# kylegrover/raymarch-algo-compare

Measured on AMD Instinct MI355X. Metric: Mrays/sec (mean iters/ray alongside), 1920x1080 Mandelbulb/Standard, higher is better.
Workload: dtype f64

## Files before the change

raymarch_algo_compare_amd/csrc/rm_kernels.h:

```cpp
#pragma once

#define RM_TABLES_IN_LDS 1

#include <hip/hip_runtime.h>
#include <stdint.h>
#include <type_traits>

#include "rm_camera.h"
#include "rm_capture.h"
#include "rm_scenes.h"
#include "rm_shape.h"
#include "rm_strategies.h"

namespace rm {

constexpr int kHistBins = 544;
constexpr int kStatsHead = 24;
constexpr int kStatsWords = kStatsHead + kHistBins;
constexpr int kQueues = 2;
constexpr int kStatsParts = 64;
constexpr int kStatsBlocks = 1 + kStatsParts;

struct FrameParams {
    CameraParams cam;
// ... 615 lines not shown
            continue;
        }

        bool park = false;
        bool consume = active;
        if constexpr (INTERLEAVE) consume = active && ready;
        if (!INTERLEAVE || __any(consume)) {
            if (consume) {
                double d;
                if constexpr (INTERLEAVE) d = Scene::value(ev);
                else d = Scene::sdf(origin + dir * s.te);
                ++nev;
            if (s.step(d, cfg)) {
                    active = false;
                    const int it = s.res.iters, h = s.res.hit;
                    a.depth[my_gi] = h ? (float)s.res.t : 0.0f;
                    a.iters[my_gi] = it;
                    a.hit[my_gi] = (uint8_t)h;
                    if (raw_out) store_raw(a, my_gi, s.res, nev);
                    acc.evals += (unsigned)nev;
                    acc.add(it, h);
                    atomicAdd(&s_hist[min(it, a.hist_bins - 1)], 1u);
                    if (a.tile_cost) {
                        const uint32_t frame = my_gi / frame_elems;
                        const uint32_t pix = my_gi - frame * frame_elems;
                        const uint32_t y = pix / (uint32_t)a.width, x = pix - y * (uint32_t)a.width;
                        atomicMax(&a.tile_cost[frame * (uint32_t)a.tiles_per_frame + (y / 4u) * (uint32_t)a.tiles_x + (x >> 6)], it);
                    }
                } else if (a.suspend_after > 0 && s.i >= a.suspend_after) {
                    park = true;
                } else if constexpr (INTERLEAVE) {
                    ready = Scene::begin(ev, origin + dir * s.te);
                }
            }
            if (a.suspend_after > 0 && __any(park)) {
                const bool parked = push_suspended(a, a.suspend_queue, park, my_gi, s, nev);
                if (parked) {
                    active = false;
                } else if (park) {
                    if constexpr (INTERLEAVE) ready = Scene::begin(ev, origin + dir * s.te);
                }
            }
        }
        if constexpr (INTERLEAVE) {
            if (active && !ready) ready = Scene::trip(ev);
        }
    }

    unsigned long long* const part = stats_part(a.stats);
    acc.flush(part);
    __syncthreads();
    for (int b = threadIdx.x; b < kHistBins; b += blockDim.x) {
        const unsigned int c = s_hist[b];
        if (c) atomicAdd(&part[kStatsHead + b], (unsigned long long)c);
    }
}


template <class Scene>
__global__ __launch_bounds__(256) void sdf_eval_kernel(const double* __restrict__ xyz, size_t n, double* __restrict__ out, const void* scene_data)
{
    rm_load_scene_data<Scene>(scene_data);
    rm_load_tables<Scene>();
    size_t i = (size_t)blockIdx.x * blockDim.x + threadIdx.x;
    if (i < n) out[i] = Scene::sdf(v3(xyz[3 * i], xyz[3 * i + 1], xyz[3 * i + 2]));
}

template <class Scene, class Strat>
__global__ __launch_bounds__(64) void march_rays_kernel(MarchCfg cfg, const double* __restrict__ origins, const double* __restrict__ dirs,
                                  size_t n, uint8_t* hit, double* t, int32_t* iters, double* final_sdf, const void* scene_data)
{
    rm_load_scene_data<Scene>(scene_data);
    rm_load_tables<Scene>();
    size_t i = (size_t)blockIdx.x * blockDim.x + threadIdx.x;
    if (i >= n) return;
    vec3 o = v3(origins[3 * i], origins[3 * i + 1], origins[3 * i + 2]);
    vec3 d = normalized(v3(dirs[3 * i], dirs[3 * i + 1], dirs[3 * i + 2]));
    Result r = march_one<Scene, Strat>(o, d, cfg);
    hit[i] = (uint8_t)r.hit; t[i] = r.t; iters[i] = r.iters; final_sdf[i] = r.final_sdf;
}

constexpr int kTeam = 3;

struct TeamXch {
    double v[2][2 * kTeam][64];
};

template <class Scene, class PartT>
__device__ __forceinline__ bool team_trip(typename Scene::Eval& ev, bool go, PartT part, int lane, TeamXch& x, int& turn)
{
    double o0 = 0.0, o1 = 0.0;
    if constexpr (std::is_same<PartT, int>::value) {
        if (go) Scene::trip_part(ev, part, o0, o1);
    } else {
        if (go) Scene::template trip_part<PartT::value>(ev, o0, o1);
    }
    double (*buf)[64] = x.v[turn & 1];
    ++turn;
    buf[2 * (int)part][lane] = o0;
    buf[2 * (int)part + 1][lane] = o1;
    __syncthreads();
    bool done = true;
    if (go) done = Scene::trip_join(ev, buf[0][lane], buf[1][lane], buf[2][lane], buf[3][lane], buf[4][lane], buf[5][lane]);
    return done;
}

template <class Scene, class = void>
struct ScenePartLoops : std::false_type {};
template <class Scene>
struct ScenePartLoops<Scene, decltype((void)Scene::kPartLoops)> : std::integral_constant<bool, Scene::kPartLoops> {};

template <int P, class Trip>
__device__ __forceinline__ void team_trips_part(bool& ready, const Trip& trip)
{
    while (__any(!ready)) {
        const bool fin = trip(std::integral_constant<int, P>(), !ready);
        if (!ready) ready = fin;
    }
}
template <class Scene, class Trip>
__device__ __forceinline__ void team_trips(int part, bool& ready, const Trip& trip)
{
    if constexpr (ScenePartLoops<Scene>::value) {
        part = __builtin_amdgcn_readfirstlane(part);
        if (part == 0) team_trips_part<0>(ready, trip);
        else if (part == 1) team_trips_part<1>(ready, trip);
        else team_trips_part<2>(ready, trip);
    } else {
        while (__any(!ready)) {
            const bool fin = trip(part, !ready);
            if (!ready) ready = fin;
        }
    }
}

template <class Scene, class Strat>
__global__ __launch_bounds__(64 * kTeam) void march_rays_team_kernel(MarchCfg cfg, const double* __restrict__ origins,
                                                                     const double* __restrict__ dirs, size_t n, uint8_t* hit,
                                                                     double* t, int32_t* iters, double* final_sdf,
                                                                     unsigned long long* busy)
{
    __shared__ TeamXch xch;
    const unsigned int nteams = (unsigned int)((n + 63) / 64);
    if (blockIdx.x >= nteams) {
        if (busy) keep_busy_until(busy, (unsigned long long)nteams, 256);
        return;
    }
    rm_load_tables<Scene>();
    const int lane = lane_id();
    const int part = (int)(threadIdx.x >> 6);
    const size_t i = (size_t)blockIdx.x * 64 + (size_t)lane;
    const bool have = i < n;
    vec3 o = v3(0.0, 0.0, 0.0), d = v3(0.0, 0.0, 1.0);
    if (have) {
        o = v3(origins[3 * i], origins[3 * i + 1], origins[3 * i + 2]);
        d = normalized(v3(dirs[3 * i], dirs[3 * i + 1], dirs[3 * i + 2]));
    }
    Strat s;
    bool done = true;
    if (have) done = s.start(cfg);
    typename Scene::Eval ev;
    int turn = 0;
    while (__any(!done)) {
        bool ready = true;
        if (!done) ready = Scene::begin(ev, o + d * s.te);
        team_trips<Scene>(part, ready, [&](auto P, bool go) { return team_trip<Scene>(ev, go, P, lane, xch, turn); });
        if (!done) done = s.step(Scene::value(ev), cfg);
    }
    if (have && part == 0) {
        hit[i] = (uint8_t)s.res.hit; t[i] = s.res.t; iters[i] = s.res.iters; final_sdf[i] = s.res.final_sdf;
    }
    if (busy && threadIdx.x == 0) __hip_atomic_fetch_add(busy, 1ull, __ATOMIC_RELAXED, __HIP_MEMORY_SCOPE_AGENT);
}

template <class Scene, class Strat, bool BATCH>
__global__ __launch_bounds__(64 * kTeam) void resume_team_kernel(const KernelArgs a, const int level)
{
    using Entry = QEntry<Strat>;
    __shared__ TeamXch xch;
    __shared__ unsigned int s_hist[kHistBins];
    __shared__ unsigned int s_base;
    const int lane = lane_id();
    const int part = (int)(threadIdx.x >> 6);
    for (int b = threadIdx.x; b < kHistBins; b += blockDim.x) s_hist[b] = 0u;
    rm_load_tables<Scene>();
    __syncthreads();

    const unsigned long long pushed = a.stats[6 + level];
    const unsigned int count = (unsigned int)min(pushed, (unsigned long long)a.queue_cap);
    const Entry* const queue = (const Entry*)a.queue[level];
    const uint32_t frame_elems = (uint32_t)a.rows * (uint32_t)a.width;
    if (a.keep_busy > 0 && (int)blockIdx.x >= a.team_wgs) {
        const unsigned long long t0 = __builtin_amdgcn_s_memrealtime();
        while (__hip_atomic_load(&a.stats[8 + level], __ATOMIC_RELAXED, __HIP_MEMORY_SCOPE_AGENT) < (unsigned long long)count &&
               __builtin_amdgcn_s_memrealtime() - t0 < 3000000ull)
            __builtin_amdgcn_s_sleep(127);
        keep_busy_until(&a.stats[12 + level], (unsigned long long)a.team_wgs, a.keep_busy);
        return;
    }

    WaveAcc acc;
    bool more = count > 0;
    bool active = false;
    uint32_t my_gi = 0;
    int nev = 0;
    vec3 origin = v3(0.0, 0.0, 0.0), dir = v3(0.0, 0.0, 0.0);
    MarchCfg lane_cfg = a.single.cfg;
    int raw_out = a.raw_outputs;
    pin_lane(raw_out);
    if constexpr (!BATCH) pin_cfg(lane_cfg);
    const MarchCfg& cfg = lane_cfg;
    Strat s;
    typename Scene::Eval ev;
    int turn = 0;

    for (;;) {
        const unsigned long long idle = __ballot(!active);
        const int nidle = __popcll(idle);
        if (more && (nidle >= a.refill_min || nidle == 64)) {
            if (part == 0 && lane == 0) s_base = (unsigned int)atomicAdd(&a.stats[8 + level], (unsigned long long)nidle);
            __syncthreads();
            const unsigned int base = (unsigned int)__builtin_amdgcn_readfirstlane((int)s_base);
            __syncthreads();
            if (base >= count) {
                more = false;
            } else if (!active) {
                const unsigned int idx = base + (unsigned int)rank_in_mask(idle);
                if (idx < count) {
                    const Entry e = queue[idx];
                    my_gi = e.gi;
                    s = e.s;
                    nev = (int)e.nev;
                    const uint32_t frame = my_gi / frame_elems;
                    const uint32_t pix = my_gi - frame * frame_elems;
                    const int y = (int)(pix / (uint32_t)a.width);
                    const int x = (int)(pix - (uint32_t)y * (uint32_t)a.width);
                    const int gy = band_row(a, y);
                    if constexpr (BATCH) {
                        const FrameParams& fp = a.frames[frame];
                        camera_ray(fp.cam, a.width, a.height, x, gy, origin, dir);
                        lane_cfg = fp.cfg;
                        lane_cfg.full = a.full;
                    } else {
                        camera_ray(a.single.cam, a.width, a.height, x, gy, origin, dir);
                    }
                    active = true;
                }
            }
        }
        if (!__any(active)) {
            if (!more) break;
            continue;
        }

        bool ready = true;
        if (active) ready = Scene::begin(ev, origin + dir * s.te);
        team_trips<Scene>(part, ready, [&](auto P, bool go) { return team_trip<Scene>(ev, go, P, lane, xch, turn); });
        bool park = false;
        if (active) {
            ++nev;
            if (!s.step(Scene::value(ev), cfg)) {
                park = a.suspend_after > 0 && s.i >= a.suspend_after;
            } else {
            active = false;
            if (part == 0) {
                const int it = s.res.iters, h = s.res.hit;
                a.depth[my_gi] = h ? (float)s.res.t : 0.0f;
                a.iters[my_gi] = it;
                a.hit[my_gi] = (uint8_t)h;
                if (raw_out) store_raw(a, my_gi, s.res, nev);
                acc.evals += (unsigned)nev;
                acc.add(it, h);
                atomicAdd(&s_hist[min(it, a.hist_bins - 1)], 1u);
                if (a.tile_cost) {
                    const uint32_t frame = my_gi / frame_elems;
                    const uint32_t pix = my_gi - frame * frame_elems;
                    const uint32_t y = pix / (uint32_t)a.width, x = pix - y * (uint32_t)a.width;
                    atomicMax(&a.tile_cost[frame * (uint32_t)a.tiles_per_frame + (y / 4u) * (uint32_t)a.tiles_x + (x >> 6)], it);
                }
            }
            }
        }
        if (a.suspend_after > 0 && __any(park)) {
            const unsigned long long m = __ballot(park);
            if (part == 0 && lane == 0) {
                const unsigned long long b64 = atomicAdd(&a.stats[6 + a.suspend_queue], (unsigned long long)__popcll(m));
                s_base = b64 > 0xffffff00ull ? 0xffffff00u : (unsigned int)b64;
            }
            __syncthreads();
            const unsigned int base = (unsigned int)__builtin_amdgcn_readfirstlane((int)s_base);
            __syncthreads();
            const unsigned long long idx = (unsigned long long)base + (unsigned long long)rank_in_mask(m);
            if (park && idx < (unsigned long long)a.queue_cap) {
                if (part == 0) {
                    Entry* e = (Entry*)a.queue[a.suspend_queue] + idx;
                    e->gi = my_gi;
                    e->nev = (uint32_t)nev;
                    e->s = s;
                }
                active = false;
            }
        }
    }

    unsigned long long* const spart = stats_part(a.stats);
    if (part == 0) acc.flush(spart);
    __syncthreads();
    for (int b = threadIdx.x; b < kHistBins; b += blockDim.x) {
        const unsigned int c = s_hist[b];
        if (c) atomicAdd(&spart[kStatsHead + b], (unsigned long long)c);
    }
    if (a.keep_busy > 0 && threadIdx.x == 0) __hip_atomic_fetch_add(&a.stats[12 + level], 1ull, __ATOMIC_RELAXED, __HIP_MEMORY_SCOPE_AGENT);
}

struct CaptureArgs {
    CameraParams cam;
    const CameraParams* cams;
    int32_t width, height, row0, rows;
    int32_t max_iterations;
    double max_distance;
    const uint8_t* hit;
    const double* t;
    const float* depth_in;
    const int32_t* iters;
    const double* final_sdf;
    const int32_t* evals;
    float* geom;
    float* normal;
    float* depth;
    float* color;
    float* evals_f;
    const void* scene_data;
};

template <class Scene> struct CaptureTables {};
template <class Scene> struct SceneTables<CaptureTables<Scene>> { static constexpr unsigned value = SceneTables<Scene>::value | TB_POW; };

template <class Scene>
__global__ __launch_bounds__(256) void capture_kernel(CaptureArgs a)
{
    rm_load_scene_data<Scene>(a.scene_data);
    rm_load_tables<CaptureTables<Scene>>();
    const size_t n = (size_t)a.rows * (size_t)a.width;
    const size_t i = (size_t)blockIdx.x * blockDim.x + threadIdx.x;
// ... 38 lines not shown
```

raymarch_algo_compare_amd/csrc/rm_pipeline.h:

```cpp
#pragma once

#include "rm_kernels.h"

namespace rm {

constexpr int kCtlStride = 16;
constexpr int kCTile = 0;
constexpr int kCReserved = 1;
constexpr int kCTaken = 3;
constexpr int kCFreshDone = 5;
constexpr int kCProdExited = 6;
constexpr int kCLeft = 7;
constexpr int kCLateStarted = 8;
constexpr int kCTeamDone = 9;
constexpr int kCtlWords = 10 * kCtlStride;
__device__ __forceinline__ unsigned long long* ctl(const KernelArgs& a, int k) { return a.ctl + k * kCtlStride; }
constexpr int kWMarkStart = 13;
constexpr int kWMarkFresh = 14;
constexpr int kWMarkProd = 15;
constexpr int kWMarkTiles = 17;
constexpr int kWMarkPush = 18;
constexpr int kWMarkPop = 19;
constexpr int kWLongPushMax = 20;
constexpr int kWLongTeamMax = 21;
// ... 55 lines not shown
            }
        }
    }
    __builtin_amdgcn_fence(__ATOMIC_ACQUIRE, "agent");
    return ok;
}

template <class Strat>
__device__ __forceinline__ bool q_push(const KernelArgs& a, int q, bool want, uint32_t gi, const Strat& s, int nev)
{
    const unsigned long long m = __ballot(want);
    if (m == 0) return false;
    unsigned long long base = 0;
    if (lane_id() == 0)
        base = __hip_atomic_fetch_add(ctl(a, kCReserved + q), (unsigned long long)__popcll(m), __ATOMIC_RELAXED,
                                      __HIP_MEMORY_SCOPE_AGENT);
    base = ((unsigned long long)(unsigned)__builtin_amdgcn_readfirstlane((int)(base >> 32)) << 32) |
           (unsigned)__builtin_amdgcn_readfirstlane((int)base);
    const unsigned long long idx = base + (unsigned long long)rank_in_mask(m);
    const bool ok = want && idx < (unsigned long long)a.queue_cap;
    static_assert(sizeof(QEntry<Strat>) % 8 == 0 && alignof(QEntry<Strat>) == 8, "entries are copied as 8-byte words");
    constexpr int NW = (int)(sizeof(QEntry<Strat>) / 8);
    constexpr int NP = (NW + 1) / 2;
    unsigned long long* const dst = (unsigned long long*)((QEntry<Strat>*)a.queue[q] + (ok ? idx : 0ull));
    unsigned long long w[NW];
    {
        QEntry<Strat> e;
        e.gi = gi;
        e.nev = (uint32_t)nev;
        e.ready = 0u;
        e.pad = a.marks ? (uint32_t)(realtime() - ~ld_relaxed(&a.stats[kWMarkStart])) : 0u;
        e.s = s;
        __builtin_memcpy(w, &e, sizeof e);
    }
    const int lane = lane_id();
    for (unsigned long long mm = __ballot(ok); mm != 0; mm &= mm - 1) {
        const int src = (int)__builtin_ctzll(mm);
        const unsigned int ilo = (unsigned int)__builtin_amdgcn_readlane((int)(unsigned int)idx, src);
        const unsigned int ihi = (unsigned int)__builtin_amdgcn_readlane((int)(unsigned int)(idx >> 32), src);
        unsigned int p0 = 0, p1 = 0, p2 = 0, p3 = 0;
#pragma unroll
        for (int p = 0; p < NP; ++p) {
            const unsigned int a0 = (unsigned int)__builtin_amdgcn_readlane((int)(unsigned int)w[2 * p], src);
            const unsigned int a1 = (unsigned int)__builtin_amdgcn_readlane((int)(unsigned int)(w[2 * p] >> 32), src);
            unsigned int a2 = 0, a3 = 0;
            if (2 * p + 1 < NW) {
                a2 = (unsigned int)__builtin_amdgcn_readlane((int)(unsigned int)w[2 * p + 1], src);
                a3 = (unsigned int)__builtin_amdgcn_readlane((int)(unsigned int)(w[2 * p + 1] >> 32), src);
            }
            if (lane == p) { p0 = a0; p1 = a1; p2 = a2; p3 = a3; }
        }
        char* const d = (char*)((QEntry<Strat>*)a.queue[q] + (((unsigned long long)ihi << 32) | ilo)) + 16 * lane;
        static_assert(std::is_base_of<StratBase, Strat>::value && __builtin_offsetof(StratBase, res) == 32 && sizeof(Result) == 24 &&
                      sizeof(QEntry<StratBase>) - sizeof(StratBase) == 16, "entry pieces 3 and 4 hold the result record");
        const bool dead = !a.full && (lane == 3 || (NW == 9 && lane == 4));
        if (lane < NP && !dead) {
            if ((NW & 1) && lane == NP - 1) {
                __hip_atomic_store((unsigned long long*)d, ((unsigned long long)p1 << 32) | p0, __ATOMIC_RELAXED, __HIP_MEMORY_SCOPE_AGENT);
            } else {
                typedef unsigned int u32x4 __attribute__((ext_vector_type(4)));
                const u32x4 v = { p0, p1, p2, p3 };
                asm volatile("global_store_dwordx4 %0, %1, off sc1" ::"v"(d), "v"(v) : "memory");
            }
        }
    }
    asm volatile("s_waitcnt vmcnt(0)" ::: "memory");
    if (ok) __hip_atomic_store((uint32_t*)(dst + 1), a.generation, __ATOMIC_RELAXED, __HIP_MEMORY_SCOPE_AGENT);
    if (a.marks && q == 1 && lane_id() == 0) atomicMax(&a.stats[kWMarkPush], realtime());
    return ok;
}


template <int TILE_PIX>
struct PipeProducerLds {
    float depth[kPipeWaves][kSlots][TILE_PIX];
    uint32_t ih[kPipeWaves][kSlots][TILE_PIX];
};
struct PipeTeamLds {
    TeamXch xch;
    unsigned int hist[kHistBins];
    unsigned int base, count, queue, done;
    unsigned int ok_lo, ok_hi;
};

__device__ __forceinline__ void store_direct(const KernelArgs& a, uint32_t gi, const Result& r, int nev, WaveAcc& acc,
                                             unsigned int* s_hist)
{
    const int it = r.iters, h = r.hit;
    a.depth[gi] = h ? (float)r.t : 0.0f;
    a.iters[gi] = it;
    a.hit[gi] = (uint8_t)h;
    if (a.raw_outputs) store_raw(a, gi, r, nev);
    acc.evals += (unsigned)nev;
    acc.add(it, h);
    atomicAdd(&s_hist[min(it, a.hist_bins - 1)], 1u);
    if (a.tile_cost) {
        const uint32_t frame_elems = (uint32_t)a.rows * (uint32_t)a.width;
        const uint32_t frame = gi / frame_elems;
        const uint32_t pix = gi - frame * frame_elems;
        const uint32_t y = pix / (uint32_t)a.width, x = pix - y * (uint32_t)a.width;
        atomicMax(&a.tile_cost[frame * (uint32_t)a.tiles_per_frame + (y / (uint32_t)a.tile_h) * (uint32_t)a.tiles_x + (x >> 6)], it);
    }
}

template <class Scene, class E>
__device__ __forceinline__ auto early_handover(const KernelArgs& a, const E& ev, int i) -> decltype(Scene::eval_trips(ev), bool())
{
    return a.early_handover > 0 && i >= a.early_handover && Scene::eval_trips(ev) >= a.early_trips;
}
template <class Scene>
__device__ __forceinline__ bool early_handover(const KernelArgs&, const NoEval&, int) { return false; }
template <class Scene, class E>
__device__ __forceinline__ bool early_handover(const KernelArgs&, const E&, long) { return false; }

template <class Scene, class Strat, int TILE_H, bool INTERLEAVE, bool BATCH>
__global__ __launch_bounds__(64 * kPipeWaves, 2) void pipeline_kernel(const KernelArgs a)
{
    static_assert(!INTERLEAVE || SceneIterative<Scene>::value, "INTERLEAVE needs Scene::Eval");
    constexpr bool TEAMS = SceneIterative<Scene>::value;
    constexpr int TILE_PIX = kTileW * TILE_H;
    using Entry = QEntry<Strat>;
    using PLds = PipeProducerLds<TILE_PIX>;
    constexpr size_t kRoleBytes = sizeof(PLds) > sizeof(PipeTeamLds) ? sizeof(PLds) : sizeof(PipeTeamLds);
    __shared__ __attribute__((aligned(16))) unsigned char s_role[kRoleBytes];
    __shared__ unsigned int s_hist[kHistBins];
    __shared__ unsigned int s_leave;

    const int lane = lane_id();
    const int wave = (int)(threadIdx.x >> 6);
    for (int b = threadIdx.x; b < kHistBins; b += blockDim.x) s_hist[b] = 0u;
    if (threadIdx.x == 0) s_leave = 0u;
    rm_load_tables<Scene>();
    __syncthreads();
    if (a.marks && threadIdx.x == 0) atomicMax(&a.stats[kWMarkStart], ~realtime());

    WaveAcc acc;
    const bool late_team = TEAMS && (int)blockIdx.x >= a.late_team_first;
    const bool team_wg = TEAMS && ((int)blockIdx.x < a.team_wgs || late_team);
    if (late_team && threadIdx.x == 0) __hip_atomic_fetch_add(ctl(a, kCLateStarted), 1ull, __ATOMIC_RELAXED, __HIP_MEMORY_SCOPE_AGENT);
    constexpr int kRole[8] = { 0, 1, 2, -1, -1, -1, -1, -1 };
    const int wave_role = !team_wg ? -2 : kRole[wave & 7];
    const bool team_role = team_wg && wave_role >= 0;
    if (team_wg) {
        PipeTeamLds& T = *reinterpret_cast<PipeTeamLds*>(s_role);
        for (int b = threadIdx.x; b < kHistBins; b += blockDim.x) T.hist[b] = 0u;
        if (threadIdx.x == 0) { T.base = T.count = T.queue = T.done = 0u; T.ok_lo = T.ok_hi = 0u; }
        __syncthreads();
    }

    if constexpr (TEAMS) {
    if (team_wg && wave_role == -1) return;
    if (team_role) {
        if (a.team_prio >= 3) __builtin_amdgcn_s_setprio(3);
        else if (a.team_prio == 2) __builtin_amdgcn_s_setprio(2);
        else if (a.team_prio == 1) __builtin_amdgcn_s_setprio(1);
        const int team = wave_role / kTeam;
        PipeTeamLds& L = reinterpret_cast<PipeTeamLds*>(s_role)[team];
        const int part = wave_role % kTeam;
        bool active = false;
        uint32_t my_gi = 0;
        uint32_t my_push = 0;
        uint32_t my_pop = 0, nev_pop = 0;
        int nev = 0;
        vec3 origin = v3(0.0, 0.0, 0.0), dir = v3(0.0, 0.0, 0.0);
        MarchCfg lane_cfg = a.single.cfg;
        if constexpr (!BATCH) pin_cfg(lane_cfg);
        const MarchCfg& cfg = lane_cfg;
        Strat s;
        typename Scene::Eval ev;
        int turn = 0;
        int since_try = 0;
        unsigned long long idle_since = 0;

        for (;;) {
            const unsigned long long idle = __ballot(!active);
            const int nidle = __popcll(idle);
            const bool look = nidle == 64 || (nidle >= a.refill_min && since_try >= a.team_retry);
            if (look) {
                since_try = 0;
                if (part == 0) {
                    unsigned int base = 0, done = 0;
                    int q = 1, cnt = 0;
                    if (lane == 0) {
                        cnt = q_claim_lane0(a, 1, nidle, base);
                        if (cnt == 0 && a.team_steal) { q = 0; cnt = q_claim_lane0(a, 0, nidle, base); }
                        if (cnt == 0 && nidle == 64) {
                            const unsigned long long ex = ld_relaxed(ctl(a, kCProdExited));
                            if (ex >= (unsigned long long)a.producer_waves && q_available(a, 1) <= 0 && q_available(a, 0) <= 0) done = 1;
                            const unsigned long long now = realtime();
                            if (idle_since == 0) idle_since = now;
                            if (!done && now - idle_since > kMaxTeamWaitTicks) { atomicMax(&a.stats[kWError], 2ull); done = 1; }
                        } else if (cnt > 0) {
                            idle_since = 0;
                            if (a.marks && q == 1) atomicMax(&a.stats[kWMarkPop], realtime());
                        }
                    }
                    cnt = __builtin_amdgcn_readfirstlane(cnt);
                    q = __builtin_amdgcn_readfirstlane(q);
                    base = (unsigned int)__builtin_amdgcn_readfirstlane((int)base);
                    unsigned long long okm = 0;
                    if (cnt > 0) {
                        const int rank = rank_in_mask(idle);
                        const bool want = !active && rank < cnt;
                        const bool got = q_wait_ready<Strat>(a, q, want, base + (unsigned int)rank);
                        okm = __ballot(want && got);
                    }
                    if (lane == 0) {
                        L.base = base; L.count = (unsigned int)cnt; L.queue = (unsigned int)q; L.done = done;
                        L.ok_lo = (unsigned int)okm; L.ok_hi = (unsigned int)(okm >> 32);
                    }
                }
                __syncthreads();
                const unsigned int base = L.base, cnt = L.count, q = L.queue, done = L.done;
                const unsigned long long okm = ((unsigned long long)L.ok_hi << 32) | (unsigned long long)L.ok_lo;
                __syncthreads();
                if (done) break;
                if (cnt > 0) {
                    if (part != 0) __builtin_amdgcn_fence(__ATOMIC_ACQUIRE, "agent");
                    const int rank = rank_in_mask(idle);
                    const bool mine = ((okm >> lane) & 1ull) != 0;
                    if (mine) {
                        const Entry* const e = (const Entry*)a.queue[q] + (base + (unsigned int)rank);
                        my_gi = e->gi;
                        nev = (int)e->nev;
                        s = e->s;
                        my_push = e->pad;
                        if (a.trace) { my_pop = (uint32_t)(realtime() - ~ld_relaxed(&a.stats[kWMarkStart])); nev_pop = (uint32_t)nev; }
                        uint32_t frame; int x, gy;
                        element_pixel(a, my_gi, frame, x, gy);
                        if constexpr (BATCH) {
                            const FrameParams& fp = a.frames[frame];
                            camera_ray(fp.cam, a.width, a.height, x, gy, origin, dir);
                            lane_cfg = fp.cfg;
                            lane_cfg.full = a.full;
                        } else {
                            camera_ray(a.single.cam, a.width, a.height, x, gy, origin, dir);
                        }
                        active = true;
                    }
                } else if (nidle == 64) {
                    __builtin_amdgcn_s_sleep(127);
                    __builtin_amdgcn_s_sleep(127);
                    continue;
                }
            }
            if (!__any(active)) continue;

            ++since_try;
            bool ready = true;
            if (active) ready = Scene::begin(ev, origin + dir * s.te);
            team_trips<Scene>(part, ready, [&](auto P, bool go) { return team_trip<Scene>(ev, go, P, lane, L.xch, turn); });
            const int live = a.trace ? __popcll(__ballot(active)) : 0;
            if (active) {
                ++nev;
                if (s.step(Scene::value(ev), cfg)) {
                    active = false;
                    if (part == 0) {
                        store_direct(a, my_gi, s.res, nev, acc, L.hist);
                        if (a.trace) {
                            const uint32_t k = atomicAdd(&a.trace[0], 1u);
                            if (k < a.trace_cap) {
                                uint32_t* const r = a.trace + 8 + 8 * (size_t)k;
                                r[0] = my_gi; r[1] = (uint32_t)s.res.iters; r[2] = my_push; r[3] = my_pop;
                                r[4] = (uint32_t)(realtime() - ~ld_relaxed(&a.stats[kWMarkStart]));
                                r[5] = nev_pop; r[6] = (uint32_t)nev; r[7] = (uint32_t)blockIdx.x | ((uint32_t)live << 16);
                            }
                        }
                        if (a.marks && s.res.iters >= kLongRay) {
                            const unsigned long long now = realtime() - ~ld_relaxed(&a.stats[kWMarkStart]);
                            atomicMax(&a.stats[kWLongPushMax], (unsigned long long)my_push);
                            atomicMax(&a.stats[kWLongPushMin], ~(unsigned long long)my_push);
                            atomicMax(&a.stats[kWLongTeamMax], now - my_push);
                            atomicMax(&a.stats[kWLongTeamMin], ~(now - my_push));
                        }
                    }
                }
            }
        }
        unsigned long long* const spart = stats_part(a.stats);
        if (part == 0) acc.flush(spart);
        __syncthreads();
        for (int b = part * 64 + lane; b < kHistBins; b += 64 * kTeam) {
            const unsigned int c = L.hist[b];
            if (c) atomicAdd(&spart[kStatsHead + b], (unsigned long long)c);
        }
        if (part == 0 && lane == 0) __hip_atomic_fetch_add(ctl(a, kCTeamDone), 1ull, __ATOMIC_RELAXED, __HIP_MEMORY_SCOPE_AGENT);
        return;
    }
    }

    PLds& L = *reinterpret_cast<PLds*>(s_role);
    float (*const s_depth)[TILE_PIX] = L.depth[wave];
    uint32_t (*const s_ih)[TILE_PIX] = L.ih[wave];
    const int ntiles = a.tiles_per_frame * a.nframes;
    const int team_wgs = TEAMS ? a.team_wgs : 0;
    const int pwave = ((int)blockIdx.x - team_wgs) * kPipeWaves + wave;
    const int park0 = a.suspend_after;
    const int park1 = (TEAMS && a.team_wgs > 0) ? a.suspend_after2 : 0;
    const bool queues = park0 > 0;
    const bool detach = a.q0_detach != 0;
    const bool may_leave = TEAMS && detach && park1 > 0 && ((int)blockIdx.x - team_wgs) < a.early_exit_wgs;
    bool leaving = false;

    int slot_tile[kSlots], slot_out[kSlots];
#pragma unroll
    for (int k = 0; k < kSlots; ++k) { slot_tile[k] = -1; slot_out[k] = 0; }
    int cur = 0;
    int pool_next = TILE_PIX;
    bool more_tiles = true;
    bool first_tile = true;
    TileGeom cg = { 0, 0, 0, 0, 0, 0, 0 };

    bool active = false;
    bool resumed = false;
    bool nopark = false;
    int my_slot = 0, my_pix = 0;
    uint32_t my_gi = 0;
    int nev = 0;
    vec3 origin = v3(0.0, 0.0, 0.0), dir = v3(0.0, 0.0, 0.0);
    MarchCfg lane_cfg = a.single.cfg;
    if constexpr (!BATCH) pin_cfg(lane_cfg);
    const MarchCfg& cfg = lane_cfg;
    int raw_out = a.raw_outputs;
    pin_lane(raw_out);
    Strat s;
    typename EvalOf<Scene, INTERLEAVE>::type ev;
    bool ready = false;
    bool dirty = true;
    bool fresh_reported = false;
    int spins = 0;
    int since_look = 0;

    for (;;) {
        if (dirty) {
        dirty = false;
        since_look = 0;
#pragma unroll
        for (int k = 0; k < kSlots; ++k) {
            const bool pool_done = (k != cur) || pool_next >= TILE_PIX;
            if (slot_tile[k] >= 0 && slot_out[k] == 0 && pool_done) {
                wave_lds_fence();
                const TileGeom g = tile_geom<TILE_H>(a, slot_tile[k]);
                const int gx = g.x0 + lane;
                const bool col_ok = lane < g.tw;
                long long bs = 0, bq = 0;
                const bool want_bv = a.block_var != nullptr;
                float* o_depth = a.depth; int32_t* o_iters = a.iters; uint8_t* o_hit = a.hit;
                pin_lane(o_depth); pin_lane(o_iters); pin_lane(o_hit);
#pragma unroll
                for (int r = 0; r < TILE_H; ++r) {
                    if (r < g.th && col_ok) {
                        const int li = r * kTileW + lane;
                        const size_t gi = g.out0 + (size_t)(g.y0 + r) * (size_t)a.width + (size_t)gx;
                        const uint32_t ih = s_ih[k][li];
                        if (ih != kSuspended) {
                            const int it = (int)(ih & 0x7fffffffu);
                            const int h = (int)(ih >> 31);
                            o_depth[gi] = s_depth[k][li];
                            o_iters[gi] = it;
                            o_hit[gi] = (uint8_t)h;
                            acc.add(it, h);
                            atomicAdd(&s_hist[min(it, a.hist_bins - 1)], 1u);
                            if (want_bv) { bs += it; bq += (long long)it * it; }
                        }
                    }
                    if ((r & 3) == 3 && want_bv) {
                        long long S = bs, Q = bq;
                        S += __shfl_xor(S, 1); Q += __shfl_xor(Q, 1);
                        S += __shfl_xor(S, 2); Q += __shfl_xor(Q, 2);
// ... 292 lines not shown
```

raymarch_algo_compare_amd/csrc/rm_scenes.h:

```cpp
#pragma once

#include "rm_core.h"

namespace rm {

enum : unsigned { TB_POW = 1u, TB_SINCOS = 2u, TB_ACOS = 4u, TB_ATAN = 8u, TB_LOG = 16u };
template <class Scene> struct SceneTables { static constexpr unsigned value = TB_POW; };
template <class Scene> struct SceneIterative { static constexpr bool value = false; };


RM_HD double sd_sphere(vec3 p, double radius) { return length(p) - radius; }

RM_HD double sd_box(vec3 p, vec3 b)
{
    vec3 q = v3(rm_fabs(p.x) - b.x, rm_fabs(p.y) - b.y, rm_fabs(p.z) - b.z);
    double outside = length(v3(py_max(q.x, 0.0), py_max(q.y, 0.0), py_max(q.z, 0.0)));
    double inside = py_min(py_max(q.x, py_max(q.y, q.z)), 0.0);
    return outside + inside;
}

RM_HD double sd_plane(vec3 p, vec3 n, double offset) { return dot(p, n) - offset; }

RM_HD double sd_cylinder(vec3 p, double radius, double half_height)
{
// ... 78 lines not shown
        double d = sd_sphere(p, 2.0);
        d = rm_fabs(d) - 0.1;
        d = rm_fabs(d) - 0.05;
        return d;
    }
};
struct SceneMenger {
    static RM_HD double sdf(vec3 p)
    {
        double d = sd_box(p, v3(1.0, 1.0, 1.0));
        double s = 1.0;
#pragma unroll
        for (int i = 0; i < 3; ++i) {
            vec3 a = v3(py_mod_pow2(p.x * s, 2.0) - 1.0, py_mod_pow2(p.y * s, 2.0) - 1.0,
                        py_mod_pow2(p.z * s, 2.0) - 1.0);
            s *= 3.0;
            vec3 r = v3(rm_fabs(1.0 - 3.0 * rm_fabs(a.x)), rm_fabs(1.0 - 3.0 * rm_fabs(a.y)),
                        rm_fabs(1.0 - 3.0 * rm_fabs(a.z)));
            double da = py_max(r.x, r.y);
            double db = py_max(r.y, r.z);
            double dc = py_max(r.z, r.x);
            double c = (py_min(da, py_min(db, dc)) - 1.0) / s;
            d = py_max(d, c);
        }
        return d;
    }
};
struct SceneMandelbulb {
    struct Eval {
        vec3 p, z;
        double dr, r;
        int32_t i;
    };
    static RM_HD bool begin(Eval& e, vec3 p)
    {
        e.p = p; e.z = p; e.dr = 1.0; e.i = 0;
        e.r = length_a(p);
        return e.r > 4.0;
    }
    static RM_HD int eval_trips(const Eval& e) { return e.i; }
    static RM_HD bool trip(Eval& e)
    {
        const double power = 8.0;
        const vec3 z = e.z;
        const double r = e.r;
        double theta = rm_acos(py_max(-1.0, py_min(1.0, z.z / py_max(r, 1e-12))));
        double phi = rm_atan2(z.y, z.x);
        double r7, zr;
        rm_pow2(r, power - 1.0, power, &r7, &zr);
        e.dr = r7 * power * e.dr + 1.0;
        theta *= power;
        phi *= power;
        double st, ct, sp, cp;
        rm_sincos(theta, &st, &ct);
        rm_sincos(phi, &sp, &cp);
        e.z = v3(zr * st * cp, zr * st * sp, zr * ct) + e.p;
        if (++e.i >= 8) return true;
        e.r = length_a(e.z);
        return e.r > 4.0;
    }
    static constexpr bool kPartLoops = true;
    template <int P>
    static RM_HD void trip_part(const Eval& e, double& o0, double& o1)
    {
        const double power = 8.0;
        if constexpr (P == 0) {
            double theta = rm_acos<true>(py_max(-1.0, py_min(1.0, e.z.z / py_max(e.r, 1e-12))));
            theta *= power;
            rm_sincos<true>(theta, &o0, &o1);
        } else if constexpr (P == 1) {
            double phi = rm_atan2<true>(e.z.y, e.z.x);
            phi *= power;
            rm_sincos<true>(phi, &o0, &o1);
        } else {
            rm_pow2(e.r, power - 1.0, power, &o0, &o1);
        }
    }
    static RM_HD void trip_part(const Eval& e, int part, double& o0, double& o1)
    {
        if (part == 0) trip_part<0>(e, o0, o1);
        else if (part == 1) trip_part<1>(e, o0, o1);
        else trip_part<2>(e, o0, o1);
    }
    static RM_HD bool trip_join(Eval& e, double st, double ct, double sp, double cp, double r7, double zr)
    {
        const double power = 8.0;
        e.dr = r7 * power * e.dr + 1.0;
        e.z = v3(zr * st * cp, zr * st * sp, zr * ct) + e.p;
        if (++e.i >= 8) return true;
        e.r = length_a(e.z);
        return e.r > 4.0;
    }
    static RM_HD double value(const Eval& e)
    {
        return 0.5 * rm_log(py_max(e.r, 1e-12)) * e.r / py_max(e.dr, 1e-12);
    }
    static RM_HD double sdf(vec3 p)
    {
        Eval e;
        bool done = begin(e, p);
        while (!done) done = trip(e);
        return value(e);
    }
};
struct SceneBadLipschitz {
    static RM_HD double sdf(vec3 p) { return (length(p) - 1.0) * 2.0; }
};
struct ScenePillars {
    static RM_HD double sdf(vec3 p)
    {
        vec3 q = v3(repeat_axis(p.x, 2.0), p.y, repeat_axis(p.z, 2.0));
        double d_pillar = sd_cylinder(q, 0.15, 3.0);
        double d_floor = sd_plane(p, v3(0.0, 1.0, 0.0), -3.0);
        return py_min(d_pillar, d_floor);
    }
};
struct SceneThinPlanes {
    static RM_HD double sdf(vec3 p)
    {
        const double spacing = 0.5;
        double py_m = py_mod_pow2(p.y + spacing * 0.5, spacing) - spacing * 0.5;
        vec3 q = v3(p.x, py_m, p.z);
        return rm_fabs(sd_plane(q, v3(0.0, 1.0, 0.0), 0.0)) - 0.01;
    }
};

#define RM_CLOUD_LIST_A(X)                                                                 \
    X(0.4253, 1.3505, 0.9373, 0.4723) X(-0.9343, -0.6794, 1.2701, 0.4257)                 \
    X(-1.6821, 1.0922, 1.0100, 0.3090) X(-0.1090, -0.6697, -0.7534, 0.4659)               \
    X(-0.8334, -0.1867, 0.0155, 0.4879) X(0.1819, 1.6847, 0.9951, 0.4789)                 \
    X(0.4154, 1.6625, -0.9680, 0.4053) X(-1.1553, 0.3826, -1.5506, 0.3120)
#define RM_CLOUD_LIST_B(X)                                                                 \
    X(-1.5787, 0.0506, -0.1149, 0.3223) X(1.4184, 0.4394, 0.0480, 0.4841)                 \
    X(-0.0106, -0.8584, -1.6599, 0.4015) X(-1.0458, 0.6529, -1.0179, 0.3197)              \
    X(-0.4436, -1.6873, 1.1222, 0.4745) X(-1.1748, -0.7902, 1.2931, 0.4211)               \
    X(0.0333, 1.1803, 0.4750, 0.4053) X(0.8220, -1.3889, 0.1399, 0.3628)
#define RM_CLOUD_LIST_C(X)                                                                 \
    X(0.0264, 1.2626, -0.4717, 0.3704) X(0.3338, -1.4985, -0.3821, 0.3327)                \
    X(-0.6017, -1.1893, 1.0755, 0.2884) X(-0.4099, 1.6277, 0.3060, 0.4728)                \
    X(0.3572, 0.4692, 0.5999, 0.3829) X(-1.1873, -0.2029, -0.8855, 0.4005)                \
    X(-0.3315, -1.3712, 1.5906, 0.3509) X(-0.9690, 0.5840, -0.6786, 0.4453)
#define RM_CLOUD_LIST(X) RM_CLOUD_LIST_A(X) RM_CLOUD_LIST_B(X) RM_CLOUD_LIST_C(X)

struct UnionEval {
    vec3 p;
    double d;
};

struct SceneSphereCloud {
    static RM_HD double sdf(vec3 p)
    {
        double d = 1e10;
#define RM_X(cx, cy, cz, r) d = py_min(d, sd_sphere(p - v3(cx, cy, cz), r));
        RM_CLOUD_LIST(RM_X)
#undef RM_X
        return d;
    }
    using Eval = UnionEval;
    static RM_HD bool begin(Eval& e, vec3 p) { e.p = p; return false; }
    static RM_HD bool trip(Eval& e) { e.d = sdf(e.p); return true; }
    static RM_HD double value(const Eval& e) { return e.d; }
    template <int P>
    static RM_HD void trip_part(const Eval& e, double& o0, double& o1)
    {
        const vec3 p = e.p;
        double d = 1e10;
// ... 144 lines not shown
```

Baseline: 272.0.

## Compute Mandelbulb distance value on the pow wave during the final team trip

Measured after the change: 268.5. -1.3%, worse.

```diff
diff --git a/raymarch_algo_compare_amd/csrc/rm_kernels.h b/raymarch_algo_compare_amd/csrc/rm_kernels.h
--- a/raymarch_algo_compare_amd/csrc/rm_kernels.h
+++ b/raymarch_algo_compare_amd/csrc/rm_kernels.h
@@ -721,21 +721,33 @@
 
 constexpr int kTeam = 3;
 
+constexpr int kChoreWave = 2;
+
 struct TeamXch {
-    double v[2][2 * kTeam][64];
+    double v[2][2 * kTeam + 1][64];
 };
 
-template <class Scene, class PartT>
-__device__ __forceinline__ bool team_trip(typename Scene::Eval& ev, bool go, PartT part, int lane, TeamXch& x, int& turn)
+template <class Scene, class = void>
+struct SceneFinalTrip : std::integral_constant<int, -1> {};
+template <class Scene>
+struct SceneFinalTrip<Scene, decltype((void)Scene::kFinalTrip)> : std::integral_constant<int, Scene::kFinalTrip> {};
+
+template <class Scene, class PartT, class FinalT = std::false_type>
+__device__ __forceinline__ bool team_trip(typename Scene::Eval& ev, bool go, PartT part, int lane, TeamXch& x, int& turn, FinalT = FinalT())
 {
     double o0 = 0.0, o1 = 0.0;
-    if constexpr (std::is_same<PartT, int>::value) {
+    double (*buf)[64] = x.v[turn & 1];
+    ++turn;
+    if constexpr (FinalT::value) {
+        static_assert(PartT::value == kChoreWave && Scene::kValuePart == kChoreWave, "the value is the chore wave's");
+        double val = 0.0;
+        if (go) val = Scene::trip_part_final(ev, o0, o1);
+        buf[2 * kTeam][lane] = val;
+    } else if constexpr (std::is_same<PartT, int>::value) {
         if (go) Scene::trip_part(ev, part, o0, o1);
     } else {
         if (go) Scene::template trip_part<PartT::value>(ev, o0, o1);
     }
-    double (*buf)[64] = x.v[turn & 1];
-    ++turn;
     buf[2 * (int)part][lane] = o0;
     buf[2 * (int)part + 1][lane] = o1;
     __syncthreads();
@@ -744,17 +756,46 @@
     return done;
 }
 
+template <class Scene>
+__device__ __forceinline__ double team_value(const typename Scene::Eval& ev, bool live, int lane, const TeamXch& x, int turn)
+{
+    if constexpr (SceneFinalTrip<Scene>::value >= 0) {
+        const bool staged = live && Scene::ended_by_count(ev);
+        const bool plain = live && !staged;
+        double d = 0.0;
+        if (staged) d = x.v[(turn - 1) & 1][2 * kTeam][lane];
+        if (__any(plain)) {
+            if (plain) d = Scene::value(ev);
+        }
+        return d;
+    } else {
+        return Scene::value(ev);
+    }
+}
+
 template <class Scene, class = void>
 struct ScenePartLoops : std::false_type {};
 template <class Scene>
 struct ScenePartLoops<Scene, decltype((void)Scene::kPartLoops)> : std::integral_constant<bool, Scene::kPartLoops> {};
 
-template <int P, class Trip>
+template <int P, class Scene, class Trip>
 __device__ __forceinline__ void team_trips_part(bool& ready, const Trip& trip)
 {
-    while (__any(!ready)) {
-        const bool fin = trip(std::integral_constant<int, P>(), !ready);
-        if (!ready) ready = fin;
+    if constexpr (P == kChoreWave && SceneFinalTrip<Scene>::value >= 0) {
+#pragma unroll 1
+        for (int k = 0; k < SceneFinalTrip<Scene>::value && __any(!ready); ++k) {
+            const bool fin = trip(std::integral_constant<int, P>(), std::false_type(), !ready);
+            if (!ready) ready = fin;
+        }
+        if (__any(!ready)) {
+            const bool fin = trip(std::integral_constant<int, P>(), std::true_type(), !ready);
+            if (!ready) ready = fin;
+        }
+    } else {
+        while (__any(!ready)) {
+            const bool fin = trip(std::integral_constant<int, P>(), std::false_type(), !ready);
+            if (!ready) ready = fin;
+        }
     }
 }
 template <class Scene, class Trip>
@@ -762,12 +803,13 @@
 {
     if constexpr (ScenePartLoops<Scene>::value) {
         part = __builtin_amdgcn_readfirstlane(part);
-        if (part == 0) team_trips_part<0>(ready, trip);
-        else if (part == 1) team_trips_part<1>(ready, trip);
-        else team_trips_part<2>(ready, trip);
+        if (part == 0) team_trips_part<0, Scene>(ready, trip);
+        else if (part == 1) team_trips_part<1, Scene>(ready, trip);
+        else team_trips_part<2, Scene>(ready, trip);
     } else {
+        static_assert(SceneFinalTrip<Scene>::value < 0, "a final trip needs per-part loops");
         while (__any(!ready)) {
-            const bool fin = trip(part, !ready);
+            const bool fin = trip(part, std::false_type(), !ready);
             if (!ready) ready = fin;
         }
     }
@@ -803,10 +845,11 @@
     while (__any(!done)) {
         bool ready = true;
         if (!done) ready = Scene::begin(ev, o + d * s.te);
-        team_trips<Scene>(part, ready, [&](auto P, bool go) { return team_trip<Scene>(ev, go, P, lane, xch, turn); });
-        if (!done) done = s.step(Scene::value(ev), cfg);
-    }
-    if (have && part == 0) {
+        team_trips<Scene>(part, ready, [&](auto P, auto F, bool go) { return team_trip<Scene>(ev, go, P, lane, xch, turn, F); });
+        const double d_ev = team_value<Scene>(ev, !done, lane, xch, turn);
+        if (!done) done = s.step(d_ev, cfg);
+    }
+    if (have && part == kChoreWave) {
         hit[i] = (uint8_t)s.res.hit; t[i] = s.res.t; iters[i] = s.res.iters; final_sdf[i] = s.res.final_sdf;
     }
     if (busy && threadIdx.x == 0) __hip_atomic_fetch_add(busy, 1ull, __ATOMIC_RELAXED, __HIP_MEMORY_SCOPE_AGENT);
@@ -894,11 +937,12 @@
 
         bool ready = true;
         if (active) ready = Scene::begin(ev, origin + dir * s.te);
-        team_trips<Scene>(part, ready, [&](auto P, bool go) { return team_trip<Scene>(ev, go, P, lane, xch, turn); });
+        team_trips<Scene>(part, ready, [&](auto P, auto F, bool go) { return team_trip<Scene>(ev, go, P, lane, xch, turn, F); });
+        const double d_ev = team_value<Scene>(ev, active, lane, xch, turn);
         bool park = false;
         if (active) {
             ++nev;
-            if (!s.step(Scene::value(ev), cfg)) {
+            if (!s.step(d_ev, cfg)) {
                 park = a.suspend_after > 0 && s.i >= a.suspend_after;
             } else {
             active = false;
diff --git a/raymarch_algo_compare_amd/csrc/rm_pipeline.h b/raymarch_algo_compare_amd/csrc/rm_pipeline.h
--- a/raymarch_algo_compare_amd/csrc/rm_pipeline.h
+++ b/raymarch_algo_compare_amd/csrc/rm_pipeline.h
@@ -161,6 +161,9 @@
     unsigned int base, count, queue, done;
     unsigned int ok_lo, ok_hi;
 };
+constexpr unsigned int kLookGo = 0u;
+constexpr unsigned int kLookDone = 1u;
+constexpr unsigned int kLookLatch = 2u;
 
 __device__ __forceinline__ void store_direct(const KernelArgs& a, uint32_t gi, const Result& r, int nev, WaveAcc& acc,
                                              unsigned int* s_hist)
@@ -200,6 +203,7 @@
     constexpr int TILE_PIX = kTileW * TILE_H;
     using Entry = QEntry<Strat>;
     using PLds = PipeProducerLds<TILE_PIX>;
+    static_assert(sizeof(PipeTeamLds) <= sizeof(PipeProducerLds<kTileW * 4>), "team block larger than the producers' staging");
     constexpr size_t kRoleBytes = sizeof(PLds) > sizeof(PipeTeamLds) ? sizeof(PLds) : sizeof(PipeTeamLds);
     __shared__ __attribute__((aligned(16))) unsigned char s_role[kRoleBytes];
     __shared__ unsigned int s_hist[kHistBins];
@@ -249,27 +253,32 @@
         typename Scene::Eval ev;
         int turn = 0;
         int since_try = 0;
+        bool latched = false;
         unsigned long long idle_since = 0;
 
         for (;;) {
             const unsigned long long idle = __ballot(!active);
             const int nidle = __popcll(idle);
-            const bool look = nidle == 64 || (nidle >= a.refill_min && since_try >= a.team_retry);
+            if (latched && nidle == 64) break;
+            const bool look = nidle == 64 || (!latched && nidle >= a.refill_min && since_try >= a.team_retry);
             if (look) {
                 since_try = 0;
-                if (part == 0) {
-                    unsigned int base = 0, done = 0;
+                if (part == kChoreWave) {
+                    unsigned int base = 0, done = kLookGo;
                     int q = 1, cnt = 0;
                     if (lane == 0) {
                         cnt = q_claim_lane0(a, 1, nidle, base);
                         if (cnt == 0 && a.team_steal) { q = 0; cnt = q_claim_lane0(a, 0, nidle, base); }
-                        if (cnt == 0 && nidle == 64) {
+                        if (cnt == 0) {
                             const unsigned long long ex = ld_relaxed(ctl(a, kCProdExited));
-                            if (ex >= (unsigned long long)a.producer_waves && q_available(a, 1) <= 0 && q_available(a, 0) <= 0) done = 1;
-                            const unsigned long long now = realtime();
-                            if (idle_since == 0) idle_since = now;
-                            if (!done && now - idle_since > kMaxTeamWaitTicks) { atomicMax(&a.stats[kWError], 2ull); done = 1; }
-                        } else if (cnt > 0) {
+                            if (ex >= (unsigned long long)a.producer_waves && q_available(a, 1) <= 0 && q_available(a, 0) <= 0)
+                                done = nidle == 64 ? kLookDone : kLookLatch;
+                            if (nidle == 64) {
+                                const unsigned long long now = realtime();
+                                if (idle_since == 0) idle_since = now;
+                                if (done == kLookGo && now - idle_since > kMaxTeamWaitTicks) { atomicMax(&a.stats[kWError], 2ull); done = kLookDone; }
+                            }
+                        } else {
                             idle_since = 0;
                             if (a.marks && q == 1) atomicMax(&a.stats[kWMarkPop], realtime());
                         }
@@ -293,9 +302,10 @@
                 const unsigned int base = L.base, cnt = L.count, q = L.queue, done = L.done;
                 const unsigned long long okm = ((unsigned long long)L.ok_hi << 32) | (unsigned long long)L.ok_lo;
                 __syncthreads();
-                if (done) break;
+                if (done == kLookDone) break;
+                if (done == kLookLatch) latched = true;
                 if (cnt > 0) {
-                    if (part != 0) __builtin_amdgcn_fence(__ATOMIC_ACQUIRE, "agent");
+                    if (part != kChoreWave) __builtin_amdgcn_fence(__ATOMIC_ACQUIRE, "agent");
                     const int rank = rank_in_mask(idle);
                     const bool mine = ((okm >> lane) & 1ull) != 0;
                     if (mine) {
@@ -328,13 +338,14 @@
             ++since_try;
             bool ready = true;
             if (active) ready = Scene::begin(ev, origin + dir * s.te);
-            team_trips<Scene>(part, ready, [&](auto P, bool go) { return team_trip<Scene>(ev, go, P, lane, L.xch, turn); });
+            team_trips<Scene>(part, ready, [&](auto P, auto F, bool go) { return team_trip<Scene>(ev, go, P, lane, L.xch, turn, F); });
+            const double d_ev = team_value<Scene>(ev, active, lane, L.xch, turn);
             const int live = a.trace ? __popcll(__ballot(active)) : 0;
             if (active) {
                 ++nev;
-                if (s.step(Scene::value(ev), cfg)) {
+                if (s.step(d_ev, cfg)) {
                     active = false;
-                    if (part == 0) {
+                    if (part == kChoreWave) {
                         store_direct(a, my_gi, s.res, nev, acc, L.hist);
                         if (a.trace) {
                             const uint32_t k = atomicAdd(&a.trace[0], 1u);
@@ -357,13 +368,13 @@
             }
         }
         unsigned long long* const spart = stats_part(a.stats);
-        if (part == 0) acc.flush(spart);
+        if (part == kChoreWave) acc.flush(spart);
         __syncthreads();
         for (int b = part * 64 + lane; b < kHistBins; b += 64 * kTeam) {
             const unsigned int c = L.hist[b];
             if (c) atomicAdd(&spart[kStatsHead + b], (unsigned long long)c);
         }
-        if (part == 0 && lane == 0) __hip_atomic_fetch_add(ctl(a, kCTeamDone), 1ull, __ATOMIC_RELAXED, __HIP_MEMORY_SCOPE_AGENT);
+        if (part == kChoreWave && lane == 0) __hip_atomic_fetch_add(ctl(a, kCTeamDone), 1ull, __ATOMIC_RELAXED, __HIP_MEMORY_SCOPE_AGENT);
         return;
     }
     }
diff --git a/raymarch_algo_compare_amd/csrc/rm_scenes.h b/raymarch_algo_compare_amd/csrc/rm_scenes.h
--- a/raymarch_algo_compare_amd/csrc/rm_scenes.h
+++ b/raymarch_algo_compare_amd/csrc/rm_scenes.h
@@ -184,6 +184,16 @@
         else if (part == 1) trip_part<1>(e, o0, o1);
         else trip_part<2>(e, o0, o1);
     }
+    static constexpr int kFinalTrip = 7;
+    static constexpr int kValuePart = 2;
+    static RM_HD bool ended_by_count(const Eval& e) { return e.i >= 8; }
+    static RM_HD double trip_part_final(const Eval& e, double& o0, double& o1)
+    {
+        const double power = 8.0;
+        rm_pow2(e.r, power - 1.0, power, &o0, &o1);
+        const double dr = o0 * power * e.dr + 1.0;
+        return 0.5 * rm_log(py_max(e.r, 1e-12)) * e.r / py_max(dr, 1e-12);
+    }
     static RM_HD bool trip_join(Eval& e, double st, double ct, double sp, double cp, double r7, double zr)
     {
         const double power = 8.0;
```
